# AdamCodd/local-hyperDB

Measured on AMD Instinct MI355X. Metric: queries/sec, N=10M d=384 fp16 top-100 (single-query stream; p50 latency alongside), higher is better.
Workload: dtype f16; 1 GPU; N=10000000 d=384 fp16 Q=1 cosine_similarity top-100, row-sharded x1; rows_per_gpu=10000000, accumulate=f32, exchange=none

## Files before the change

local-hyperdb_amd/csrc/hdb_api.hip:

```cpp
#include "hdb_common.h"
#include "hdb_quant.h"
#include "hdb_ws.h"
#include "hdb_plan.h"
#include "../../include/hyperdb_hip.h"
#include <string>
#include <cmath>
#include <cstring>
#include <cstdio>
#include <algorithm>
#include <vector>
#include <chrono>
#include <atomic>

static thread_local std::string g_err;
static int fail(int code, const std::string& msg) { g_err = msg; return code; }
#define HIP_TRY(expr)                                                                              \
    do {                                                                                           \
        hipError_t e_ = (expr);                                                                    \
        if (e_ != hipSuccess)                                                                      \
            return fail(HDB_ERR_HIP, std::string(#expr) + ": " + hipGetErrorString(e_));           \
    } while (0)
#define LAUNCH_TRY(expr)                                                                           \
    do {                                                                                           \
        int e_ = (expr);                                                                           \
// ... 59 lines not shown
    int64_t profile = 0;
    std::vector<hipEvent_t> ev_pool;
    size_t ev_used = 0;
};

static int ensure_ws(hdb_index* ix, size_t bytes) {
    if (bytes <= ix->ws_bytes) return HDB_OK;
    if (ix->ws) { HIP_TRY(hipDeviceSynchronize()); HIP_TRY(hipFree(ix->ws)); ix->ws = nullptr; ix->ws_bytes = 0; }
    bytes = align_up(bytes + (bytes >> 2), 1 << 20);
    HIP_TRY(hipMalloc((void**)&ix->ws, bytes));
    ix->ws_bytes = bytes;
    return HDB_OK;
}
template <typename WS, typename... Ext>
static int ws_lay(hdb_index* ix, WS& w, Ext... ext) {
    const int rc = ensure_ws(ix, ws_bytes_for<WS>(ext...));
    if (rc) return rc;
    Bump b(ix->ws, ix->ws_bytes);
    w.lay(b, ext...);
    if (b.off > b.cap) return fail(HDB_ERR_NOMEM, "workspace: a layout ran past the size it reported");
    return HDB_OK;
}

extern "C" int hdb_version(void) { return 105; }
extern "C" const char* hdb_last_error(void) { return g_err.c_str(); }

static int build_caches(hdb_index* ix, hipStream_t st) {
    if (ix->n > ix->cache_rows) {
        if (ix->inv_norm) { HIP_TRY(hipDeviceSynchronize()); HIP_TRY(hipFree(ix->inv_norm)); HIP_TRY(hipFree(ix->sqnorm)); }
        const int64_t rows = ix->n + ix->n / 4 + 64;
        HIP_TRY(hipMalloc((void**)&ix->inv_norm, rows * sizeof(float)));
        HIP_TRY(hipMalloc((void**)&ix->sqnorm, rows * sizeof(float)));
        ix->cache_rows = rows;
    }
    HIP_TRY(hipMemsetAsync(ix->nan_flag, 0, sizeof(int), st));
    if (ix->n > 0) LAUNCH_TRY(hdb_launch_rownorm(ix->V, ix->n, ix->d, ix->dtype, ix->inv_norm, ix->sqnorm, ix->nan_flag, st));
    ix->flags_host = -1;
    ix->bits_valid = false; ix->bits_done = 0;
    ix->pscale_valid = false; ix->pscale_done = 0;
    ix->build_stream = st;
    return HDB_OK;
}

static double quant_gamma(int d) {
    const double u = std::ldexp(1.0, -24), m = (double)(d + 8) * u;
    return m / (1.0 - m) * (1.0 + std::ldexp(1.0, -20));
}
// ... 339 lines not shown
    else if (!strcmp(name, "dyn_heavy")) ix->opt.dyn_heavy = value;
    else if (!strcmp(name, "fused_timeout_us")) ix->opt.fused_timeout_us = std::max<int64_t>(1, value);
    else if (!strcmp(name, "bits_fused")) ix->opt.bits_fused = value;
    else if (!strcmp(name, "bits_local")) ix->opt.bits_local = value;
    else if (!strcmp(name, "fused_max_q")) ix->opt.fused_max_q = value;
    else if (!strcmp(name, "f32_min_q")) ix->opt.f32_min_q = value;
    else if (!strcmp(name, "f32_split")) ix->opt.f32_split = value;
    else if (!strcmp(name, "f32_split_min_q")) ix->opt.f32_split_min_q = value;
    else if (!strcmp(name, "bf16_ks_min_q")) ix->opt.bf16_ks_min_q = value;
    else if (!strcmp(name, "f8_ks_min_q")) ix->opt.f8_ks_min_q = value < 0 ? -1 : value;
    else if (!strcmp(name, "f8_lds_min_q")) ix->opt.f8_lds_min_q = value < 0 ? -1 : value;
    else if (!strcmp(name, "bf16_quant")) ix->opt.bf16_quant = value ? 1 : 0;
    else if (!strcmp(name, "f8_lds_waves")) { if (value == 0 || value == 4 || value == 8) ix->opt.f8_lds_waves = value; }
    else if (!strcmp(name, "bits_max_q")) ix->opt.bits_max_q = value;
    else if (!strcmp(name, "use_quant")) ix->opt.use_quant = value;
    else if (!strcmp(name, "quant_min_n")) ix->opt.quant_min_n = value;
    else if (!strcmp(name, "auto_quant")) ix->opt.auto_quant = value;
    else if (!strcmp(name, "quant_batch_min_n")) ix->opt.quant_batch_min_n = value;
    else if (!strcmp(name, "quant_batch_kernel")) ix->opt.quant_batch_kernel = value ? 1 : 0;
    else if (!strcmp(name, "quant_max_k")) ix->opt.quant_max_k = std::max<int64_t>(1, std::min<int64_t>(value, 128));
    else if (!strcmp(name, "use_plane")) ix->opt.use_plane = value;
    else if (!strcmp(name, "plane_min_n")) ix->opt.plane_min_n = value;
    else if (!strcmp(name, "plane_cap_rows")) ix->opt.plane_cap_rows = std::max<int64_t>(0, value);
    else if (!strcmp(name, "use_subset")) ix->opt.use_subset = value;
    else if (!strcmp(name, "subset_min_n")) ix->opt.subset_min_n = value < 0 ? -1 : value;
    else if (!strcmp(name, "subset_ratio")) ix->opt.subset_ratio = value < 0 ? -1 : std::max<int64_t>(1, value);
    else if (!strcmp(name, "profile")) { ix->profile = value; ix->ev_used = 0; }
    else if (!strcmp(name, "host_timing_reset")) { ix->ht_pre_ns = ix->ht_launch_ns = ix->ht_wait_ns = ix->ht_calls = ix->ht_attr_ns = 0; }
    else return fail(HDB_ERR_ARG, std::string("hdb_set_option: unknown option ") + name);
    return HDB_OK;
}

extern "C" int hdb_get_stat(hdb_index* ix, const char* name, int64_t* value) {
    if (!ix || !name || !value) return fail(HDB_ERR_ARG, "hdb_get_stat: null argument");
    if (!strcmp(name, "sample_rows")) *value = ix->st.sample_rows;
    else if (!strcmp(name, "sample_m")) *value = ix->st.sample_m;
    else if (!strcmp(name, "path")) *value = ix->st.path;
    else if (!strcmp(name, "chunks")) *value = ix->st.chunks;
    else if (!strcmp(name, "mfma")) *value = ix->st.mfma;
    else if (!strcmp(name, "f32_split")) *value = ix->st.f32s;
    else if (!strcmp(name, "f8_lds")) *value = ix->st.f8_lds;
    else if (!strcmp(name, "f8_lds_min_q")) *value = f8_lds_first_q(ix->opt, ix->dtype, ix->d);
    else if (!strcmp(name, "host_direct")) *value = ix->st_host_direct;
    else if (!strcmp(name, "fused")) *value = ix->st.fused;
    else if (!strcmp(name, "local")) *value = ix->st.local;
    else if (!strcmp(name, "cand_cap")) *value = HDB_CAND_CAP;
    else if (!strcmp(name, "quant")) *value = ix->st.quant;
    else if (!strcmp(name, "quant_auto")) *value = (ix->qmode == HDB_QUANT_I8 && ix->qauto) ? 1 : 0;
    else if (!strcmp(name, "quant_bytes")) *value = ix->qmode == HDB_QUANT_I8 ? ix->n * (int64_t)(ix->qP + 12) : 0;
    else if (!strcmp(name, "plane")) *value = ix->st.plane;
    else if (!strcmp(name, "subset")) *value = ix->st.subset;
    else if (!strcmp(name, "subset_rows")) *value = ix->subset_m;
    else if (!strcmp(name, "plane_bytes")) *value = (ix->qmode == HDB_QUANT_I8 && ix->pnib) ? ix->n * (int64_t)plane_row_bytes(ix->qP) : 0;
    else if (!strcmp(name, "plane_survivors") || !strcmp(name, "plane_overflows")) {
        int h[HDB_QSTAT_WORDS] = {0, 0, 0, 0};
        if (ix->qstat) {
            HIP_TRY(hipSetDevice(ix->device));
            HIP_TRY(hipDeviceSynchronize());
            HIP_TRY(hipMemcpy(h, ix->qstat, sizeof(h), hipMemcpyDeviceToHost));
        }
        *value = name[6] == 's' ? (ix->st.plane ? (int64_t)(uint32_t)h[1] : 0) : (int64_t)(uint32_t)h[2];
    }
    else if (!strcmp(name, "quant_cands")) {
        int h = 0;
        if (ix->st.quant && ix->qstat) {
            HIP_TRY(hipSetDevice(ix->device));
            HIP_TRY(hipDeviceSynchronize());
            HIP_TRY(hipMemcpy(&h, ix->qstat, sizeof(int), hipMemcpyDeviceToHost));
        }
        *value = h;
    }
    else if (!strcmp(name, "quant_cands_min") || !strcmp(name, "quant_cands_median")) {
        int64_t v = 0;
// ... 211 lines not shown
    const size_t crow = (size_t)nq * HDB_CAND_CAP;
    const int nsub = p.nsub;
    rc = quant_query_prep(ix, (const float*)dev_Q, nq, w, mflavour, ix->qstat, nsub ? w.cnt : nullptr, pl_cnt, st);
    if (rc) return rc;
    QuantArgs a; quant_base_args(ix, a, w.qcodes, w.qaux, w.qinv, metric, nq);
    a.ntiles = sp.s_tiles; a.tile_stride = sp.s_stride; a.scores = w.sbuf; a.ld = sp.ld_s;
    a.wmax = w.wmax; a.nsub = nsub; a.thr_out = w.thr;
    a.pl_hi = use_pl ? reinterpret_cast<float*>(w.pl_list) : nullptr;
    if (use_pl && (!a.pl_hi || sp.s_rows > (int64_t)quant_hi_cap(ix, nq))) return fail(HDB_ERR_ARG, "quant_topk: no list for the sampled rows");
    LAUNCH_TRY(hdb_launch_quant_scan(&a, 0, (int)ix->opt.max_blocks, st));
    if (!nsub) LAUNCH_TRY(hdb_launch_sample_thr(w.sbuf, sp.s_rows, sp.ld_s, nq, m, w.thr, w.cnt, nullptr, st));
    a.ntiles = (n + 15) / 16; a.tile_stride = 1; a.scores = nullptr; a.ld = 0;
    a.thr = w.thr; a.cnt = w.cnt; a.cand = w.cand; a.cap = HDB_CAND_CAP;
    const bool has_bias = ix->bias != nullptr || ix->mask != nullptr;
    if (mflavour) {
        a.V = (const char*)ix->V; a.row_bytes = ix->d * 2; a.G = w.G;
        a.ginv = metric == HDB_COSINE ? w.ginv : nullptr; a.gbias = has_bias ? w.gbias : nullptr;
    }
    prof_begin(ix, st);
    if (use_pl) {
        a.pl_nib = ix->pnib; a.pl_bit = ix->pbit; a.pl_rec = ix->prec; a.pl_units = ix->pU;
        a.pl_cnt = pl_cnt; a.pl_cap = p.pl_cap;
        a.pl_s_tiles = (uint32_t)sp.s_tiles; a.pl_s_stride = (uint32_t)sp.s_stride;
        LAUNCH_TRY(hdb_launch_quant_plane_scan(&a, 0, (int)ix->opt.max_blocks, st));
    } else {
        LAUNCH_TRY(hdb_launch_quant_scan(&a, 1, (int)ix->opt.max_blocks, st));
    }
    prof_end(ix, st);
    if (mflavour) {
        ScanArgs s; memset(&s, 0, sizeof(s));
        s.V = w.G; s.n = (int64_t)crow; s.d = ix->d; s.Q = dev_Q; s.metric = metric; s.inv_norm = w.ginv; s.qinv = w.qinv;
        s.bias = has_bias ? w.gbias : nullptr; s.mask = nullptr; s.nq = nq;
        s.tile_stride = 1; s.ntiles = (int64_t)crow / hdb_mfma_tile_rows(ix->dtype, ix->d); s.cap = HDB_CAND_CAP;
        s.scores = w.gsc; s.ld = (int64_t)crow;
        LAUNCH_TRY(hdb_launch_mfma_scan(&s, ix->dtype, 0, nq, w.q16, w.ginv, w.qsq, w.qscl, (int)ix->opt.max_blocks, (int)ix->opt.mfma_variant, st, nullptr));
    } else {
        LAUNCH_TRY(hdb_launch_quant_rescore(ix->V, ix->d, ix->dtype, (const float*)dev_Q, nq, metric, ix->inv_norm, w.qinv, ix->bias, ix->mask,
                                            w.cand, w.cnt, HDB_CAND_CAP, st));
    }
    LAUNCH_TRY(hdb_launch_quant_finalize(w.cand, w.cnt, HDB_CAND_CAP, nq, (uint32_t)k, kk, ix->row_base, dev_idx, dev_score, dev_status, w.qnan,
                                         w.qaux, w.thr, ix->qstat, mflavour ? w.cand : nullptr, w.gsc, (int64_t)crow, st));
    return HDB_OK;
}

extern "C" int hdb_debug_quant_bounds(hdb_index* ix, const float* dev_q, int metric, float* dev_hi, float* dev_hi5, void* stream) {
    if (!ix || !dev_q || !dev_hi || !dev_hi5) return fail(HDB_ERR_ARG, "hdb_debug_quant_bounds: null argument");
    if (metric != HDB_DOT && metric != HDB_COSINE) return fail(HDB_ERR_ARG, "hdb_debug_quant_bounds: dot or cosine");
    if (ix->qmode != HDB_QUANT_I8 || !ix->pnib || ix->n < 1) return fail(HDB_ERR_UNSUPPORTED, "hdb_debug_quant_bounds: the index has no 5-bit plane");
    HIP_TRY(hipSetDevice(ix->device));
    hipStream_t st = (hipStream_t)stream;
    QuantWs w;
    int rc = quant_ws_lay(ix, w, 1, quant_hi_cap(ix, 1), true);
    if (rc) return rc;
    rc = quant_query_prep(ix, dev_q, 1, w, ix->qauto, nullptr, nullptr, nullptr, st);
    if (rc) return rc;
    QuantArgs a; quant_base_args(ix, a, w.qcodes, w.qaux, w.qinv, metric, 1);
    a.ntiles = (ix->n + 15) / 16; a.tile_stride = 1;
    a.pl_nib = ix->pnib; a.pl_bit = ix->pbit; a.pl_rec = ix->prec; a.pl_units = ix->pU;
    a.dbg = dev_hi;
    LAUNCH_TRY(hdb_launch_quant_scan_one(&a, 2, (int)ix->opt.max_blocks, st));
    a.dbg = dev_hi5;
    LAUNCH_TRY(hdb_launch_quant_plane_scan(&a, 1, (int)ix->opt.max_blocks, st));
    return HDB_OK;
}

static int quant_batch_topk(hdb_index* ix, const TopkArgs& c, const TopkPlan& p) {
    const void* dev_Q = c.Q; const int32_t nq = c.nq, k = c.k; const int metric = c.metric; hipStream_t st = c.st;
    int64_t* dev_idx = c.idx; float* dev_score = c.score; int32_t* dev_status = c.status;
    const uint32_t kk = p.kk;
    const int64_t n = ix->n;
    const int P = ix->qP;
    const uint32_t m = HDB_QB_SAMPLE_M;
    const QuantSample sp = p.qs;
    const int64_t s_tiles = sp.s_tiles, s_stride = sp.s_stride, s_rows = sp.s_rows, ld_s = sp.ld_s;
    const int cq_max = p.cq_max;
    QuantBatchWs w;
    const int rc = quant_batch_ws_lay(ix, w, cq_max);
    if (rc) return rc;
    const int64_t wld = quant_batch_wld();
    float* const qinv = w.qinv; float* const qsq = w.qsq; int* const qnan = w.qnan; float* const qscl = w.qscl;
    int8_t* const qcodes = w.qcodes; float* const qaux = w.qaux; float* const thr = w.thr; uint32_t* const cnt = w.cnt;
    unsigned long long* const cand = w.cand; void* const q16 = w.q16; float* const wbuf = w.wbuf;
    for (int q0 = 0; q0 < nq; q0 += cq_max) {
        const int cq = std::min(cq_max, nq - q0);
        const float* Qc = (const float*)dev_Q + (size_t)q0 * ix->d;
// ... 673 lines not shown
```

local-hyperdb_amd/csrc/hdb_caps.h:

```cpp
#pragma once
#include "../../include/hyperdb_hip.h"

static inline int hdb_scan_auto_blocks(int dtype, int row_bytes, bool vec, bool wide_rows) {
    if (dtype == HDB_F8E4M3 && vec && (row_bytes == 256 || row_bytes == 384 || row_bytes == 512)) {
        const int b = 512 * 768 / row_bytes;
        return b < 1024 ? b : 1024;
    }
    return wide_rows ? 256 : 512;
}

#define HDB_KS_MAX_SLICES 8
struct KsGeom {
    int slices;
    int width[HDB_KS_MAX_SLICES];
    int off[HDB_KS_MAX_SLICES];
};
static inline KsGeom ks_list(int elem_bytes, int n0, int w0, int n1 = 0, int w1 = 0) {
    KsGeom g = {};
    int at = 0;
    for (int s = 0; s < n0 + n1 && s < HDB_KS_MAX_SLICES; ++s) {
        g.width[s] = s < n0 ? w0 : w1; g.off[s] = at * elem_bytes;
        at += g.width[s];
    }
    g.slices = n0 + n1;
// ... 137 lines not shown
#endif
#define HDB_BITS_MAXW 512
static inline int hdb_bits_fused_supported(int metric, int nq, int W, uint32_t kk) {
    return (metric == HDB_HAMMING || metric == HDB_JACCARD) && nq >= 1 && nq <= 4 && W <= HDB_BITS_MAXW && kk <= 128;
}
static inline int hdb_bits_fused_blocks(int64_t ntiles, int cus, int max_blocks) {
    int blocks = cus;
    const int64_t items = ntiles * 4;
    if ((int64_t)blocks * HDB_BITS_THREADS > items) blocks = (int)((items + HDB_BITS_THREADS - 1) / HDB_BITS_THREADS);
    if (max_blocks > 0 && max_blocks < blocks) blocks = max_blocks;
    if (blocks < 1) blocks = 1;
    return blocks;
}
static inline bool hdb_bits_fused_local(int blocks, uint32_t kk) { return (int64_t)blocks >= 2 * (int64_t)kk; }

static inline int hdb_l1_tile_supported(int dtype, int d) {
    if (dtype == HDB_F16) return d == 128 || d == 256 || d == 384 || d == 512 || d == 640 || d == 768;
    if (dtype == HDB_F32) return d == 128 || d == 256 || d == 384 || d == 512 || d == 768;
    return 0;
}

static inline int hdb_quant_scan_blocks(int64_t ntiles, int max_blocks) { return hdb_grid_for(ntiles, 4, max_blocks > 0 ? max_blocks : 1024); }
static inline int hdb_quant_plane_units(int P) { return (P + 31) / 32; }
struct HdbSkipPos { uint32_t w, o; };
struct HdbSkipStep { uint32_t dw, dn, step; };
__host__ __device__ __forceinline__ uint32_t hdb_plane_skip_count(uint32_t ntiles, uint32_t s_tiles) { return ntiles - s_tiles; }
__host__ __device__ __forceinline__ HdbSkipStep hdb_plane_skip_step(uint32_t step, uint32_t stride) {
    const uint32_t m = stride - 1u;
    HdbSkipStep s;
    s.dw = m ? step / m : 0u; s.dn = m ? step % m : 0u; s.step = step;
    return s;
}
__host__ __device__ __forceinline__ HdbSkipPos hdb_plane_skip_start(uint32_t tp, uint32_t s_tiles, uint32_t stride) {
    const uint32_t m = stride - 1u;
    HdbSkipPos p;
    const uint32_t w = m ? tp / m : s_tiles;
    if (w < s_tiles) { p.w = w; p.o = tp - w * m; }
    else { p.w = s_tiles; p.o = tp - s_tiles * m; }
    return p;
}
__host__ __device__ __forceinline__ void hdb_plane_skip_advance(HdbSkipPos& p, const HdbSkipStep& s, uint32_t s_tiles, uint32_t stride) {
    if (p.w >= s_tiles) { p.o += s.step; return; }
    const uint32_t m = stride - 1u;
    p.w += s.dw; p.o += s.dn;
    if (p.o >= m) { p.o -= m; ++p.w; }
    if (p.w >= s_tiles) { p.o += (p.w - s_tiles) * m; p.w = s_tiles; }
// ... 20 lines not shown
```

local-hyperdb_amd/csrc/hdb_launch.h:

```cpp
#pragma once
#include <stddef.h>
#include <stdint.h>

struct ScanArgs;
struct FusedArgs;
struct BatchArgs;
struct BitsArgs;
struct QuantArgs;

#define HDB_ANYD_DECL(name) int name(const ScanArgs* args, int dpad, int mode, int nq_launch, const void* q, const float* sqnorm, \
                                     const float* qsq, const float* qscl, int blocks, void* stream)
#define HDB_GEOM_DECL(name) int name(const ScanArgs* args, int mode, int nq_launch, const void* q16, const float* sqnorm, \
                                     const float* qsq, const float* qscl, int blocks, int variant, void* stream, const BatchArgs* f)

extern "C" {
int hdb_launch_scan(const ScanArgs* args, int dtype, int mode, int nq_launch, int max_blocks, void* stream);
int hdb_launch_list_rows(unsigned long long* cand, const uint32_t* cnt, uint32_t cap, int nq, const int64_t* rows, int64_t m, void* stream);
int hdb_launch_rownorm(const void* V, int64_t n, int d, int dtype, float* inv_norm, float* sqnorm, int* nan_flag, void* stream);
int hdb_launch_qprep(const void* Q, int nq, int d, bool f64, float* qinv, float* qsq, int* qnan, void* q16, float* qscl, void* stream);
int hdb_launch_qprep2(const void* Q, int nq, int d, bool f64, float* qinv, float* qsq, int* qnan, void* q16, float* qscl,
                      float* thr_init, uint32_t* cnt_init, uint32_t* qbits, int W, void* stream);
int hdb_launch_signpack(const void* V, int64_t n, int d, int dtype, int64_t row0, uint32_t* bits, void* stream);
int hdb_launch_qsign(const void* Q, int nq, int d, bool f64, int W, uint32_t* qbits, void* stream);
int hdb_launch_hamming(const ScanArgs* args, int mode, int nq_launch, const uint32_t* bits, int64_t npad, int W,
// ... 72 lines not shown
int hdb_launch_mfma_kslice_f8_lds(const ScanArgs* a, int dslice, int mode, int nq_launch, const void* q, const float* sqnorm,
                                  const float* qsq, int blocks, void* stream);
int hdb_launch_mfma_kslice_f8_lds_wide(const ScanArgs* a, int dslice, int mode, int nq_launch, const void* q, const float* sqnorm,
                                       const float* qsq, int blocks, void* stream);
HDB_ANYD_DECL(hdb_launch_mfma_anyd_a); HDB_ANYD_DECL(hdb_launch_mfma_anyd_b);
HDB_ANYD_DECL(hdb_launch_mfma_anyd_c); HDB_ANYD_DECL(hdb_launch_mfma_anyd_d);
HDB_ANYD_DECL(hdb_launch_mfma_anyd_e); HDB_ANYD_DECL(hdb_launch_mfma_anyd_f);

size_t hdb_mfma_fused_ctl_bytes(void);
int hdb_launch_mfma_fused(const ScanArgs* args, int dtype, const FusedArgs* fa, int max_blocks, void* stream);
int hdb_launch_mfma_fused_wide(const ScanArgs* args, const FusedArgs* fa, int blocks, void* stream);
int hdb_launch_bits_fused(const BitsArgs* args, int jaccard, int max_blocks, void* stream);
int hdb_launch_l1_tile(const ScanArgs* args, int dtype, int mode, int nq_launch, int max_blocks, void* stream);

int hdb_launch_quant_rows(const void* V, int64_t n, int d, int dtype, int P, int8_t* codes, float* aux, int* nan_flag, double gamma,
                          void* stream);
int hdb_launch_quant_gather(const int8_t* codes, const float* aux, const int64_t* rows, int64_t m, int P, int8_t* codes_out,
                            float* aux_out, void* stream);
int hdb_launch_quant_qprep(const float* Q, int nq, int d, int P, int8_t* qcodes, float* qaux, int* stat, uint32_t* pl_cnt, void* stream);
int hdb_launch_quant_qprep_m(const float* Q, int nq, int d, int P, float* qinv, float* qsq, int* qnan, void* q16, float* qscl,
                             int8_t* qcodes, float* qaux, int* stat, uint32_t* cnt_init, uint32_t* pl_cnt, void* stream);
int hdb_launch_quant_plane_rows(const int8_t* codes, const float* aux, int64_t row0, int64_t m, int d, int P, uint8_t* nib, uint32_t* bitw,
                                float* rec, void* stream);
int hdb_launch_quant_plane_scan(const QuantArgs* args, int dbg, int max_blocks, void* stream);
int hdb_launch_quant_scan(const QuantArgs* args, int mode, int max_blocks, void* stream);
int hdb_launch_quant_scan_one(const QuantArgs* args, int mode, int max_blocks, void* stream);
int hdb_launch_quant_rescore(const void* V, int d, int dtype, const float* Q, int nq, int metric, const float* inv_norm,
                             const float* qinv, const float* bias, const uint8_t* mask, unsigned long long* cand,
                             const uint32_t* cnt, uint32_t cap, void* stream);
int hdb_launch_quant_finalize(const unsigned long long* cand, const uint32_t* cnt, uint32_t cap, int nq, uint32_t k, uint32_t kk,
                              int64_t row_base, int64_t* idx_out, float* score_out, int32_t* status, const int* qnan,
                              const float* qaux, const float* thr, int* stat, unsigned long long* cand_rw, const float* sc, int64_t ld,
                              void* stream);

int hdb_launch_qb_scan(const QuantArgs* args, int mode, float* wstat, int64_t wld, int max_blocks, void* stream);
int hdb_launch_qb_thr(const float* vals, int64_t n, int64_t ld, int nq, uint32_t m, float* thr, void* stream);
int hdb_launch_qb_rescore(const void* V, int d, const void* q16, const float* qscl, const float* qinv, const float* inv_norm,
                          const float* bias, const uint8_t* mask, int metric, unsigned long long* cand, const uint32_t* cnt,
                          uint32_t cap, int nq, void* stream);
}
```

local-hyperdb_amd/csrc/hdb_plan.h:

```cpp
#pragma once
#include "hdb_ws.h"
#include <algorithm>

struct hdb_options {
    int64_t max_blocks = 0;
    int64_t force_exact = 0;
    int64_t sample_target = 0;
    int64_t mfma_min_q = 1;
    int64_t use_mfma = 1;
    int64_t exact_bytes = (int64_t)1 << 30;
    int64_t bits_fused = 1;
    int64_t bits_local = 1;
    int64_t fused_max_q = -1;
    int64_t f32_min_q = -1;
    int64_t f32_split = 1;
    int64_t f32_split_min_q = -1;
    int64_t bf16_ks_min_q = -1;
    int64_t f8_ks_min_q = 0;
    int64_t f8_lds_min_q = 0;
    int64_t bf16_quant = 0;
    int64_t f8_lds_waves = 0;
    int64_t bits_max_q = -1;
    int64_t host_direct = 1;
    int64_t dyn_tiles = 1;
// ... 1 lines not shown
    int64_t dyn_heavy = 0;
    int64_t host_poll = 1;
    int64_t use_fused = 1;
    int64_t use_local = 1;
    int64_t local_m = 0;
    int64_t local_max_tiles = 4;
    int64_t local_small = 0;
    int64_t local_max_q = 1;
    int64_t use_l1_tile = 1;
    int64_t l1_packed = 1;
    int64_t use_batch1 = 1;
    int64_t fused_timeout_us = 2000;
    int64_t finalize_threads = 1024;
    int64_t mfma_variant = 16;
    int64_t use_quant = 1;
    int64_t quant_min_n = -1;
    int64_t quant_max_k = 128;
    int64_t auto_quant = 1;
    int64_t quant_batch_min_n = -1;
    int64_t quant_batch_kernel = 1;
    int64_t use_plane = 1;
    int64_t plane_min_n = -1;
    int64_t plane_cap_rows = 0;
    int64_t use_subset = 1;
    int64_t subset_min_n = -1;
    int64_t subset_ratio = -1;
};

struct TopkFacts {
    int64_t n; int32_t d; int dtype;
    int qmode;
    bool qauto;
    bool qauto_declined;
    bool plane_present, plane_declined;
    bool has_mask, has_bias;
    int cus;
    int64_t subset_m;
};
struct TopkCall { int32_t nq, k; int metric; bool has_status, exact; };

enum TopkPath {
    HDB_PATH_EMPTY,
    HDB_PATH_QUANT,
    HDB_PATH_QUANT_BATCH,
    HDB_PATH_FUSED,
    HDB_PATH_BITS1,
    HDB_PATH_BATCH1,
    HDB_PATH_FULL_SORT,
    HDB_PATH_PIPELINE
};
struct TopkStats { int64_t sample_rows = 0, sample_m = 0, path = 0, chunks = 0, mfma = 0, fused = 0, local = 0, f32s = 0, quant = 0, plane = 0, subset = 0, f8_lds = 0; };
struct TopkPlan {
    TopkPath path = HDB_PATH_EMPTY;
    uint32_t kk = 0; int W = 0;
    bool bits = false, pearson = false;
    bool exact = false, small = false, mfma = false, f32s = false, ksplit = false, l1tile = false, local = false;
    bool f8_lds = false;
    bool subset = false;
    bool prep = false, fold_small = false, q16_in_prep = false, f16_queries = false, mask_fold = false;
    int tile_rows = 16;
    int64_t s_tiles = 0, s_stride = 1, s_rows = 0, ld_s = 0, ld_n = 0; uint32_t m = 0;
    int cq_max = 1;
    int64_t ld_scores = 0, ld_ks = 0, sort_n = 0;
    uint32_t local_slot = 0, local_m = 0;
    int bits_local = 0;
    int npass = 4;
    bool mflavour = false, build_needed = false, plane_wanted = false;
    bool qb_int8 = false;
    int P = 0, nsub = 0; uint32_t pl_cap = 0;
    QuantSample qs = {0, 1, 0, 0};
    TopkStats stats;
    bool shadow() const { return path == HDB_PATH_QUANT || path == HDB_PATH_QUANT_BATCH; }
    bool single_launch() const { return path == HDB_PATH_FUSED || path == HDB_PATH_BITS1 || path == HDB_PATH_BATCH1; }
};

#define HDB_FUSED_MAXQ_RULE 4
static inline bool is_bits_metric(int metric) { return metric == HDB_HAMMING || metric == HDB_JACCARD; }

static inline void sample_plan(int64_t n, int64_t sample_target, uint32_t kk, int nq, int tile_rows, bool coarse, int64_t& tiles, int64_t& stride, uint32_t& m) {
    int64_t T = sample_target > 0 ? sample_target : (kk <= 128 ? (nq >= 32 ? 1024 : 2048) : 4096);
    if (coarse && sample_target <= 0) T /= 2;
    m = kk <= 128 ? 8u : (kk <= 512 ? 64u : 256u);
    int64_t rows = (int64_t)((double)m * (double)n / (double)T);
    rows = std::max<int64_t>(rows, 16 * (int64_t)m);
    tiles = (rows + tile_rows - 1) / tile_rows;
    const int64_t all_tiles = n / tile_rows;
    tiles = std::min(tiles, all_tiles);
    stride = std::max<int64_t>(1, all_tiles / std::max<int64_t>(tiles, 1));
}

static inline int64_t quant_min_rows(int dtype) {
    return dtype == HDB_F16 ? 1250000 : dtype == HDB_BF16 ? 1000000 : 500000;
// ... 8 lines not shown
static inline bool plane_wanted(int d, const hdb_options& o) { return plane_possible(d) && o.use_plane; }

static inline int64_t quant_batch_rule(int d, int nq) {
    int64_t rows = 0;
    if (d == 384) rows = nq <= 16 ? 3000000 : nq <= 24 ? 5000000 : 0;
    else if (d == 512) rows = nq <= 16 ? 10000000 : 0;
    return rows > 0 ? std::max<int64_t>(rows, HDB_QUANT_AUTO_MIN_ROWS) : 0;
}
static inline int64_t quant_batch_wld() { return (int64_t)align_up((size_t)hdb_qb_slots(512, 1), 4); }

static inline bool auto_quant_call(const TopkFacts& ix, const hdb_options& o, const TopkCall& c, bool mfma, bool exact, bool small) {
    return o.auto_quant && o.use_quant && mfma && ix.dtype == HDB_F16 && (ix.qmode == HDB_QUANT_NONE || ix.qauto) && !exact && !small &&
           c.has_status && c.k <= o.quant_max_k && c.k <= 128 && (c.metric == HDB_DOT || c.metric == HDB_COSINE) &&
           !(ix.qmode == HDB_QUANT_NONE && ix.qauto_declined);
}

static inline void plan_quant(TopkPlan& p, const TopkFacts& ix, const hdb_options& o, const TopkCall& c, bool mflavour) {
    p.path = HDB_PATH_QUANT; p.mflavour = mflavour; p.build_needed = ix.qmode != HDB_QUANT_I8;
    p.P = (int)align_up((size_t)ix.d, 16);
    p.qs = quant_call_sample(ix.n, ix.d, p.kk);
    p.plane_wanted = c.nq == 1 && (c.metric == HDB_DOT || c.metric == HDB_COSINE) && plane_wanted(ix.d, o) && !ix.plane_declined &&
                     ix.n >= (o.plane_min_n >= 0 ? o.plane_min_n : (int64_t)HDB_PLANE_MIN_ROWS);
    p.pl_cap = plane_list_cap(o, ix.n);
    if (mflavour) {
        p.nsub = 4 * hdb_quant_scan_blocks(p.qs.s_tiles, (int)o.max_blocks);
        if (p.nsub < 1024 || p.nsub > HDB_QUANT_NSUB_MAX) p.nsub = 0;
    }
    p.stats.quant = 1; p.stats.path = 1; p.stats.mfma = mflavour ? 1 : 0; p.stats.plane = p.plane_wanted ? 1 : 0;
    p.stats.sample_rows = p.qs.s_rows; p.stats.sample_m = 16; p.stats.chunks = 1;
}
static inline void plan_quant_batch(TopkPlan& p, const TopkFacts& ix, const hdb_options& o, const TopkCall& c) {
    p.path = HDB_PATH_QUANT_BATCH; p.mflavour = true; p.build_needed = ix.qmode != HDB_QUANT_I8;
    p.P = (int)align_up((size_t)ix.d, 16);
    p.qs = quant_batch_sample(ix.n);
    p.cq_max = std::min<int>(c.nq, 256);
    p.qb_int8 = o.quant_batch_kernel != 0;
    p.stats.quant = 1; p.stats.path = 1; p.stats.mfma = 1;
    p.stats.sample_rows = p.qs.s_rows; p.stats.sample_m = HDB_QB_SAMPLE_M; p.stats.chunks = (c.nq + p.cq_max - 1) / p.cq_max;
}

#define HDB_SUBSET_RATIO 4
#define HDB_SUBSET_MIN_ROWS 50000
static inline bool subset_metric(int metric) {
    return metric == HDB_DOT || metric == HDB_COSINE || metric == HDB_EUCLIDEAN || metric == HDB_MANHATTAN || metric == HDB_PEARSON;
}
static inline bool subset_rule(const TopkFacts& ix, const hdb_options& o, const TopkCall& c) {
    if (ix.subset_m <= 0 || !o.use_subset || !subset_metric(c.metric) || c.nq < 1) return false;
    if (ix.n < (o.subset_min_n >= 0 ? o.subset_min_n : (int64_t)HDB_SUBSET_MIN_ROWS)) return false;
    const int64_t ratio = o.subset_ratio >= 1 ? std::min<int64_t>(o.subset_ratio, (int64_t)1 << 30) : (int64_t)HDB_SUBSET_RATIO;
    return ix.subset_m <= ix.n / (((int64_t)c.nq + 3) / 4 * ratio);
}
// ... 143 lines not shown
```

local-hyperdb_amd/csrc/hdb_quant.hip:

```cpp
#include "hdb_common.h"
#include "hdb_quant.h"
#include "hdb_finalize.h"
#include "../../include/hyperdb_hip.h"

__device__ __forceinline__ float hq_up(double x) {
    x = x * (1.0 + 0x1p-40);
    float f = (float)x;
    if ((double)f < x) f = nextafterf(f, INFINITY);
    return f;
}

__device__ __forceinline__ float hq_f(__half v) { return __half2float(v); }
__device__ __forceinline__ float hq_f(hdb_bf16 v) { return hdb_bf16_to_f(v); }
__device__ __forceinline__ float hq_f(float v) { return v; }

template <typename T> struct HqElem;
template <> struct HqElem<__half> { static constexpr int EPC = 8; };
template <> struct HqElem<hdb_bf16> { static constexpr int EPC = 8; };
template <> struct HqElem<float> { static constexpr int EPC = 4; };

__device__ __forceinline__ void hq_unpack(const uint4& raw, float (&x)[8], __half*) {
    const __half2* h = reinterpret_cast<const __half2*>(&raw);
#pragma unroll
    for (int i = 0; i < 4; ++i) { float2 f = __half22float2(h[i]); x[2 * i] = f.x; x[2 * i + 1] = f.y; }
// ... 538 lines not shown
    extern __shared__ __attribute__((aligned(16))) char smem[];
    int4* qs = reinterpret_cast<int4*>(smem);
    __shared__ int part[4][2][64 * J];
    __shared__ HqStage stage;
    __shared__ uint32_t queue[4][HQ_PL_QUEUE];
    __shared__ uint32_t surv_cnt;
    const int U = a.pl_units, nch = a.P >> 4;
    if (threadIdx.x < 4) stage.cnt[threadIdx.x] = 0u;
    if (threadIdx.x == 0) surv_cnt = 0u;
    for (int i = threadIdx.x; i < 2 * U; i += 256) qs[i] = i < nch ? reinterpret_cast<const int4*>(a.qcodes)[i] : make_int4(0, 0, 0, 0);
    const float* qo = a.qaux;
    const float q_s = qo[HDB_QQ_S], q_n = qo[HDB_QQ_N], q_d = qo[HDB_QQ_D], q_cn = qo[HDB_QQ_CN];
    const int q_cs = (int)qo[HDB_QQ_CS];
    const bool q_bad = qo[HDB_QQ_BAD] != 0.f;
    const bool cosine = a.metric == HDB_COSINE;
    const float q_inv = cosine ? a.qinv[0] : 1.f;
    float thr1[1] = {(!DBG && a.nsub == 0) ? a.thr[0] : 0.f};
    __syncthreads();
    if (!DBG && a.nsub > 0) hq_fold_thr<1>(a, thr1);
    const float q_thr = thr1[0];

    const int lane = threadIdx.x & 63, wave = __builtin_amdgcn_readfirstlane(threadIdx.x >> 6);
    const int npieces = 16 * U;
    int qw[J][8];
    auto load_qw = [&]() {
#pragma unroll
        for (int j = 0; j < J; ++j) {
            const int f = lane + 64 * j;
            const int unit = f < npieces ? f % U : 0;
            const int4 x = qs[2 * unit], y = qs[2 * unit + 1];
            qw[j][0] = x.x; qw[j][1] = x.y; qw[j][2] = x.z; qw[j][3] = x.w;
            qw[j][4] = y.x; qw[j][5] = y.y; qw[j][6] = y.z; qw[j][7] = y.w;
        }
    };
    load_qw();
    const float absmin = 0x1p-100f * (float)(a.d + 8);
    typedef unsigned int u32x4 __attribute__((ext_vector_type(4)));
    typedef float f32x4 __attribute__((ext_vector_type(4)));
    const int64_t ntiles = a.ntiles;
    const int et = lane >> 4, er = lane & 15;
    int qn = 0;
    uint32_t nsurv = 0u;
    auto drain = [&](int base, int m) {
        const QuantArgs& a = hq_args_in_memory();
        HqQuery<1> qc;
        qc.s[0] = q_s; qc.n[0] = q_n; qc.d[0] = q_d; qc.sq[0] = 0.f; qc.inv[0] = q_inv; qc.bad[0] = q_bad;
        int ln = lane;
        asm volatile("" : "+v"(ln));
        const int g = ln >> 4, l16 = ln & 15;
        int64_t rr[4];
#pragma unroll
        for (int u = 0; u < 4; ++u) rr[u] = 4 * g + u < m ? (int64_t)queue[wave][base + 4 * g + u] : a.n;
        const int own = 4 * g + hdb_owned_row(l16);
        const int64_t row = own < m ? (int64_t)queue[wave][base + own] : a.n;
        hq_rows4_bounds<1, 0, 1>(a, qs, qc, rr, l16, row, [&](int, float, float hi, bool masked) {
            if (!masked && !q_bad && hi >= q_thr) hq_emit(stage, 0, hi, row);
        });
    };
// ... 24 lines not shown
            for (int j = 0; j < J; ++j) {
                if (ln < pieces_left - 64 * j) {
                    nv[tt][j] = __builtin_nontemporal_load(reinterpret_cast<const u32x4*>(nb + (uint32_t)ln * 16u) + 64 * j);
                    bv[tt][j] = __builtin_nontemporal_load(bb + (uint32_t)ln + 64 * j);
                } else {
                    nv[tt][j] = u32x4{0u, 0u, 0u, 0u};
                    bv[tt][j] = 0u;
                }
            }
        }
        const int64_t row = (et ? tl[1] : tl[0]) * 16 + er;
        const bool rvalid = lane < 32 && row < a.n;
        f32x4 rc = f32x4{0.f, 0.f, 0.f, 0.f};
        float invn = 1.f, bias = 0.f;
        bool masked = false;
        if (rvalid) {
            rc = __builtin_nontemporal_load(reinterpret_cast<const f32x4*>(a.pl_rec) + row);
            if (cosine) invn = a.inv_norm[row];
            if (a.bias) bias = a.bias[row];
            if (a.mask) masked = !a.mask[row];
        }
        __builtin_amdgcn_sched_barrier(0);
#pragma unroll
        for (int tt = 0; tt < 2; ++tt) {
#pragma unroll
            for (int j = 0; j < J; ++j) {
                const uint32_t bw = bv[tt][j];
                const uint32_t w4[4] = {nv[tt][j].x, nv[tt][j].y, nv[tt][j].z, nv[tt][j].w};
                int s = 0;
#pragma unroll
                for (int i = 0; i < 4; ++i) {
                    const uint32_t lo = ((w4[i] << 1) & 0x1E1E1E1Eu) | ((bw >> (2 * i)) & 0x01010101u);
                    const uint32_t hi = ((w4[i] >> 3) & 0x1E1E1E1Eu) | ((bw >> (2 * i + 1)) & 0x01010101u);
                    s = __builtin_amdgcn_sdot4((int)lo, qw[j][2 * i], s, false);
                    s = __builtin_amdgcn_sdot4((int)hi, qw[j][2 * i + 1], s, false);
                }
                part[wave][tt][lane + 64 * j] = s;
            }
        }
        __builtin_amdgcn_fence(__ATOMIC_RELEASE, "wavefront");
        __builtin_amdgcn_wave_barrier();
        __builtin_amdgcn_fence(__ATOMIC_ACQUIRE, "wavefront");
        int S = 0;
        if (lane < 32)
            for (int i = 0; i < U; ++i) S += part[wave][et][er * U + i];
        __builtin_amdgcn_fence(__ATOMIC_RELEASE, "wavefront");
        __builtin_amdgcn_wave_barrier();
        float hi5 = -INFINITY;
        const bool dead = !rvalid || masked || q_bad;
        if (!dead) {
            const float fc = (float)(8 * S - 124 * q_cs);
            const float Uf = q_cn * rc.w;
            float ch = fc + Uf, cl = fc - Uf;
            ch = ch + (fabsf(ch) * 0x1p-20f + 1.f);
            cl = cl - (fabsf(cl) * 0x1p-20f + 1.f);
            const float k = q_s * rc.x;
            const float A5 = k * ch, Al = k * cl;
            const float Amax = fmaxf(fabsf(A5), fabsf(Al));
            const float c0 = (q_n * rc.y + q_d * rc.z) * (1.f + 0x1p-10f);
            const float B5 = c0 + fabsf(A5) * 0x1p-10f + absmin;
            const float Bmax = c0 + Amax * 0x1p-10f + absmin;
// ... 4 lines not shown
            const float Z = mM + fabsf(bias);
            float h = X;
            if (a.bias) h += bias;
            hi5 = h + (Z * 0x1p-18f + 4e-30f);
            if (hi5 != hi5) hi5 = INFINITY;
        }
        if (DBG) {
            if (rvalid) a.dbg[row] = hi5;
            continue;
        }
        const bool keep = !dead && !(hi5 < q_thr);
        const unsigned long long km = __ballot(keep);
        if (km == 0ull) continue;
        if (keep) queue[wave][qn + __popcll(km & ((1ull << lane) - 1ull))] = (uint32_t)row;
        const int nk = __popcll(km);
        qn += nk; nsurv += (uint32_t)nk;
        __builtin_amdgcn_fence(__ATOMIC_RELEASE, "wavefront");
        __builtin_amdgcn_wave_barrier();
        __builtin_amdgcn_fence(__ATOMIC_ACQUIRE, "wavefront");
        if (qn >= 16) {
            do { qn -= 16; drain(qn, 16); } while (qn >= 16);
            __builtin_amdgcn_fence(__ATOMIC_RELEASE, "wavefront");
            __builtin_amdgcn_wave_barrier();
            asm volatile("" ::: "memory");
            load_qw();
        }
    }
    if (!DBG) {
        if (s_tiles != 0u) {
            const QuantArgs& am = hq_args_in_memory();
            const uint32_t nslots = s_tiles * 16u, dslot = (uint32_t)gridDim.x * 256u;
            uint32_t cbase = ((uint32_t)blockIdx.x * 4u + (uint32_t)wave) * 64u;
            float hnext = cbase + lane < nslots ? am.pl_hi[cbase + lane] : 0.f;
#pragma unroll 1
            for (; cbase < nslots; cbase += dslot) {
                const uint32_t slot = cbase + lane;
                const float hi = hnext;
                hnext = slot + dslot < nslots ? am.pl_hi[slot + dslot] : 0.f;
                const int64_t row = hdb_tile_index((int64_t)(slot >> 4), (int64_t)s_stride) * 16 + (slot & 15u);
                bool keep = slot < nslots && !q_bad && !(hi < q_thr);
                if (keep && am.mask) keep = am.mask[row] != 0;
                const unsigned long long km = __ballot(keep);
#pragma unroll 1
                for (int h = 0; h < 2; ++h) {
                    const uint32_t kh = (uint32_t)(km >> (32 * h));
                    if (kh == 0u) continue;
                    if (keep && (lane >> 5) == h) queue[wave][qn + __popc(kh & ((1u << (lane & 31)) - 1u))] = (uint32_t)row;
                    const int nk = __popc(kh);
// ... 172 lines not shown
extern "C" int hdb_launch_quant_scan(const QuantArgs* args, int mode, int max_blocks, void* stream) {
    const QuantArgs& a = *args;
    if (a.nq < 1 || a.nq > 4 || (a.P & 15) != 0) return (int)hipErrorInvalidValue;
    const size_t lds = (size_t)a.nq * a.P;
    const int blocks = hdb_quant_scan_blocks(a.ntiles, max_blocks);
    if (a.nsub != 0 && (a.nsub > HDB_QUANT_NSUB_MAX || !a.wmax || (mode == 0 ? a.nsub != 4 * blocks : !a.thr_out))) return (int)hipErrorInvalidValue;
    if (mode == 0) hq_launch_scan_mode<0>(a, blocks, lds, (hipStream_t)stream);
    else {
        if (!hq_copy_args_ok(a)) return (int)hipErrorInvalidValue;
        hq_launch_scan_mode<1>(a, blocks, lds, (hipStream_t)stream);
    }
    return (int)hipGetLastError();
}

extern "C" int hdb_launch_quant_plane_rows(const int8_t* codes, const float* aux, int64_t row0, int64_t m, int d, int P, uint8_t* nib,
                                           uint32_t* bitw, float* rec, void* stream) {
    if (m <= 0) return 0;
    const int U = hdb_quant_plane_units(P);
    if (U > 16 || (P & 15) != 0) return (int)hipErrorInvalidValue;
    hipLaunchKernelGGL(hdb_quant_plane_rows_kernel, dim3(hdb_grid_for(m, 16, 8192)), dim3(256), 0, (hipStream_t)stream, codes, aux, row0, m, d,
                       P, U, nib, bitw, rec);
    return (int)hipGetLastError();
}
extern "C" int hdb_launch_quant_plane_scan(const QuantArgs* args, int dbg, int max_blocks, void* stream) {
    const QuantArgs& a = *args;
    const int U = a.pl_units;
    if (a.nq != 1 || U < 1 || U > 16 || U != hdb_quant_plane_units(a.P) || (a.metric != HDB_DOT && a.metric != HDB_COSINE)) return (int)hipErrorInvalidValue;
    if (!dbg && a.nsub != 0 && (a.nsub > HDB_QUANT_NSUB_MAX || !a.wmax || !a.thr_out)) return (int)hipErrorInvalidValue;
    if (!dbg && (!a.cnt || !a.cand || !a.pl_cnt || !hq_copy_args_ok(a))) return (int)hipErrorInvalidValue;
    if (a.ntiles < 0 || a.ntiles > 0x10000000) return (int)hipErrorInvalidValue;
    if (!dbg && a.pl_s_tiles != 0u && (!a.pl_hi || a.pl_s_stride < 1u || (uint64_t)a.pl_s_tiles * a.pl_s_stride > (uint64_t)a.ntiles)) return (int)hipErrorInvalidValue;
    const size_t lds = (size_t)U * 32;
    const int64_t nwalk = a.ntiles - (dbg ? 0 : (int64_t)a.pl_s_tiles);
    const int blocks = hdb_grid_for((nwalk + 1) / 2, 4, max_blocks > 0 ? max_blocks : 1024);
    hipStream_t st = (hipStream_t)stream;
    const int J = (U + 3) / 4;
#define HQ_PLANE(J_) do { if (dbg) hipLaunchKernelGGL((hdb_quant_plane_scan_kernel<J_, true>), dim3(blocks), dim3(256), lds, st, a); \
                          else hipLaunchKernelGGL((hdb_quant_plane_scan_kernel<J_, false>), dim3(blocks), dim3(256), lds, st, a); } while (0)
    if (J == 1) HQ_PLANE(1); else if (J == 2) HQ_PLANE(2); else if (J == 3) HQ_PLANE(3); else HQ_PLANE(4);
#undef HQ_PLANE
    return (int)hipGetLastError();
}
extern "C" int hdb_launch_quant_scan_one(const QuantArgs* args, int mode, int max_blocks, void* stream) {
    const QuantArgs& a = *args;
    if (a.nq != 1 || (a.P & 15) != 0 || a.nsub != 0 || mode != 2 || !a.dbg) return (int)hipErrorInvalidValue;
    const size_t lds = (size_t)a.P;
    const int blocks = hdb_quant_scan_blocks(a.ntiles, max_blocks);
    const int nj = ((a.P >> 4) + 15) >> 4;
    hipStream_t st = (hipStream_t)stream;
#define HQ_ONE(NJ_) hipLaunchKernelGGL((hdb_quant_scan_kernel<2, 1, NJ_>), dim3(blocks), dim3(256), lds, st, a)
    if (nj == 1) HQ_ONE(1); else if (nj == 2) HQ_ONE(2); else if (nj == 3) HQ_ONE(3); else HQ_ONE(0);
#undef HQ_ONE
    return (int)hipGetLastError();
}

extern "C" int hdb_launch_quant_rescore(const void* V, int d, int dtype, const float* Q, int nq, int metric, const float* inv_norm,
                                        const float* qinv, const float* bias, const uint8_t* mask, unsigned long long* cand,
                                        const uint32_t* cnt, uint32_t cap, void* stream) {
    hipStream_t st = (hipStream_t)stream;
// ... 39 lines not shown
```

Measured before the change: 1997 queries/s.

## Size plane-scan grid per CU and load query words from LDS per use

```diff
diff --git a/local-hyperdb_amd/csrc/hdb_api.hip b/local-hyperdb_amd/csrc/hdb_api.hip
--- a/local-hyperdb_amd/csrc/hdb_api.hip
+++ b/local-hyperdb_amd/csrc/hdb_api.hip
@@ -105,7 +105,7 @@
     return HDB_OK;
 }
 
-extern "C" int hdb_version(void) { return 105; }
+extern "C" int hdb_version(void) { return 106; }
 extern "C" const char* hdb_last_error(void) { return g_err.c_str(); }
 
 static int build_caches(hdb_index* ix, hipStream_t st) {
@@ -491,6 +491,7 @@
     else if (!strcmp(name, "use_plane")) ix->opt.use_plane = value;
     else if (!strcmp(name, "plane_min_n")) ix->opt.plane_min_n = value;
     else if (!strcmp(name, "plane_cap_rows")) ix->opt.plane_cap_rows = std::max<int64_t>(0, value);
+    else if (!strcmp(name, "plane_wg_per_cu")) ix->opt.plane_wg_per_cu = std::max<int64_t>(0, std::min<int64_t>(value, 8));
     else if (!strcmp(name, "use_subset")) ix->opt.use_subset = value;
     else if (!strcmp(name, "subset_min_n")) ix->opt.subset_min_n = value < 0 ? -1 : value;
     else if (!strcmp(name, "subset_ratio")) ix->opt.subset_ratio = value < 0 ? -1 : std::max<int64_t>(1, value);
@@ -518,6 +519,7 @@
     else if (!strcmp(name, "quant_auto")) *value = (ix->qmode == HDB_QUANT_I8 && ix->qauto) ? 1 : 0;
     else if (!strcmp(name, "quant_bytes")) *value = ix->qmode == HDB_QUANT_I8 ? ix->n * (int64_t)(ix->qP + 12) : 0;
     else if (!strcmp(name, "plane")) *value = ix->st.plane;
+    else if (!strcmp(name, "plane_blocks")) *value = ix->st.plane_blocks;
     else if (!strcmp(name, "subset")) *value = ix->st.subset;
     else if (!strcmp(name, "subset_rows")) *value = ix->subset_m;
     else if (!strcmp(name, "plane_bytes")) *value = (ix->qmode == HDB_QUANT_I8 && ix->pnib) ? ix->n * (int64_t)plane_row_bytes(ix->qP) : 0;
@@ -775,7 +777,7 @@
         a.pl_nib = ix->pnib; a.pl_bit = ix->pbit; a.pl_rec = ix->prec; a.pl_units = ix->pU;
         a.pl_cnt = pl_cnt; a.pl_cap = p.pl_cap;
         a.pl_s_tiles = (uint32_t)sp.s_tiles; a.pl_s_stride = (uint32_t)sp.s_stride;
-        LAUNCH_TRY(hdb_launch_quant_plane_scan(&a, 0, (int)ix->opt.max_blocks, st));
+        LAUNCH_TRY(hdb_launch_quant_plane_scan(&a, 0, p.pl_blocks, st));
     } else {
         LAUNCH_TRY(hdb_launch_quant_scan(&a, 1, (int)ix->opt.max_blocks, st));
     }
@@ -813,7 +815,7 @@
     a.dbg = dev_hi;
     LAUNCH_TRY(hdb_launch_quant_scan_one(&a, 2, (int)ix->opt.max_blocks, st));
     a.dbg = dev_hi5;
-    LAUNCH_TRY(hdb_launch_quant_plane_scan(&a, 1, (int)ix->opt.max_blocks, st));
+    LAUNCH_TRY(hdb_launch_quant_plane_scan(&a, 1, hdb_quant_plane_dbg_blocks(a.ntiles, (int)ix->opt.max_blocks), st));
     return HDB_OK;
 }
 
diff --git a/local-hyperdb_amd/csrc/hdb_caps.h b/local-hyperdb_amd/csrc/hdb_caps.h
--- a/local-hyperdb_amd/csrc/hdb_caps.h
+++ b/local-hyperdb_amd/csrc/hdb_caps.h
@@ -183,6 +183,23 @@
 
 static inline int hdb_quant_scan_blocks(int64_t ntiles, int max_blocks) { return hdb_grid_for(ntiles, 4, max_blocks > 0 ? max_blocks : 1024); }
 static inline int hdb_quant_plane_units(int P) { return (P + 31) / 32; }
+static constexpr int hdb_quant_plane_j(int U) { return (U + 3) / 4; }
+#define HDB_PLANE_WAVES {8, 8, 7, 5}
+#define HDB_PLANE_WG_PER_CU {4, 4, 3, 2}
+static constexpr int hdb_quant_plane_waves(int J) { constexpr int t[4] = HDB_PLANE_WAVES; return t[J < 1 ? 0 : J > 4 ? 3 : J - 1]; }
+static constexpr int hdb_quant_plane_wg_per_cu(int J) { constexpr int t[4] = HDB_PLANE_WG_PER_CU; return t[J < 1 ? 0 : J > 4 ? 3 : J - 1]; }
+static_assert(hdb_quant_plane_wg_per_cu(1) >= 1 && hdb_quant_plane_wg_per_cu(1) <= hdb_quant_plane_waves(1) &&
+              hdb_quant_plane_wg_per_cu(2) >= 1 && hdb_quant_plane_wg_per_cu(2) <= hdb_quant_plane_waves(2) &&
+              hdb_quant_plane_wg_per_cu(3) >= 1 && hdb_quant_plane_wg_per_cu(3) <= hdb_quant_plane_waves(3) &&
+              hdb_quant_plane_wg_per_cu(4) >= 1 && hdb_quant_plane_wg_per_cu(4) <= hdb_quant_plane_waves(4),
+              "a default grid of the plane pass asks for more waves per SIMD than its kernel is compiled for");
+static inline int hdb_quant_plane_blocks(int64_t nwalk, int J, int cus, int wg_per_cu, int max_blocks) {
+    const int per_cu = wg_per_cu >= 1 ? (wg_per_cu < 8 ? wg_per_cu : 8) : hdb_quant_plane_wg_per_cu(J);
+    int64_t limit = (int64_t)per_cu * (cus > 0 ? cus : 1);
+    if (max_blocks > 0 && max_blocks < limit) limit = max_blocks;
+    return hdb_grid_for((nwalk + 1) / 2, 4, (int)limit);
+}
+static inline int hdb_quant_plane_dbg_blocks(int64_t ntiles, int max_blocks) { return hdb_grid_for((ntiles + 1) / 2, 4, max_blocks > 0 ? max_blocks : 1024); }
 struct HdbSkipPos { uint32_t w, o; };
 struct HdbSkipStep { uint32_t dw, dn, step; };
 __host__ __device__ __forceinline__ uint32_t hdb_plane_skip_count(uint32_t ntiles, uint32_t s_tiles) { return ntiles - s_tiles; }
diff --git a/local-hyperdb_amd/csrc/hdb_launch.h b/local-hyperdb_amd/csrc/hdb_launch.h
--- a/local-hyperdb_amd/csrc/hdb_launch.h
+++ b/local-hyperdb_amd/csrc/hdb_launch.h
@@ -118,7 +118,7 @@
                              int8_t* qcodes, float* qaux, int* stat, uint32_t* cnt_init, uint32_t* pl_cnt, void* stream);
 int hdb_launch_quant_plane_rows(const int8_t* codes, const float* aux, int64_t row0, int64_t m, int d, int P, uint8_t* nib, uint32_t* bitw,
                                 float* rec, void* stream);
-int hdb_launch_quant_plane_scan(const QuantArgs* args, int dbg, int max_blocks, void* stream);
+int hdb_launch_quant_plane_scan(const QuantArgs* args, int dbg, int blocks, void* stream);
 int hdb_launch_quant_scan(const QuantArgs* args, int mode, int max_blocks, void* stream);
 int hdb_launch_quant_scan_one(const QuantArgs* args, int mode, int max_blocks, void* stream);
 int hdb_launch_quant_rescore(const void* V, int d, int dtype, const float* Q, int nq, int metric, const float* inv_norm,
diff --git a/local-hyperdb_amd/csrc/hdb_plan.h b/local-hyperdb_amd/csrc/hdb_plan.h
--- a/local-hyperdb_amd/csrc/hdb_plan.h
+++ b/local-hyperdb_amd/csrc/hdb_plan.h
@@ -47,6 +47,7 @@
     int64_t use_plane = 1;
     int64_t plane_min_n = -1;
     int64_t plane_cap_rows = 0;
+    int64_t plane_wg_per_cu = 0;
     int64_t use_subset = 1;
     int64_t subset_min_n = -1;
     int64_t subset_ratio = -1;
@@ -74,7 +75,7 @@
     HDB_PATH_FULL_SORT,
     HDB_PATH_PIPELINE
 };
-struct TopkStats { int64_t sample_rows = 0, sample_m = 0, path = 0, chunks = 0, mfma = 0, fused = 0, local = 0, f32s = 0, quant = 0, plane = 0, subset = 0, f8_lds = 0; };
+struct TopkStats { int64_t sample_rows = 0, sample_m = 0, path = 0, chunks = 0, mfma = 0, fused = 0, local = 0, f32s = 0, quant = 0, plane = 0, subset = 0, f8_lds = 0, plane_blocks = 0; };
 struct TopkPlan {
     TopkPath path = HDB_PATH_EMPTY;
     uint32_t kk = 0; int W = 0;
@@ -93,6 +94,7 @@
     bool mflavour = false, build_needed = false, plane_wanted = false;
     bool qb_int8 = false;
     int P = 0, nsub = 0; uint32_t pl_cap = 0;
+    int pl_blocks = 0;
     QuantSample qs = {0, 1, 0, 0};
     TopkStats stats;
     bool shadow() const { return path == HDB_PATH_QUANT || path == HDB_PATH_QUANT_BATCH; }
@@ -147,11 +149,15 @@
     p.plane_wanted = c.nq == 1 && (c.metric == HDB_DOT || c.metric == HDB_COSINE) && plane_wanted(ix.d, o) && !ix.plane_declined &&
                      ix.n >= (o.plane_min_n >= 0 ? o.plane_min_n : (int64_t)HDB_PLANE_MIN_ROWS);
     p.pl_cap = plane_list_cap(o, ix.n);
+    if (p.plane_wanted)
+        p.pl_blocks = hdb_quant_plane_blocks((ix.n + 15) / 16 - p.qs.s_tiles, hdb_quant_plane_j(hdb_quant_plane_units(p.P)), ix.cus,
+                                             (int)o.plane_wg_per_cu, (int)o.max_blocks);
     if (mflavour) {
         p.nsub = 4 * hdb_quant_scan_blocks(p.qs.s_tiles, (int)o.max_blocks);
         if (p.nsub < 1024 || p.nsub > HDB_QUANT_NSUB_MAX) p.nsub = 0;
     }
     p.stats.quant = 1; p.stats.path = 1; p.stats.mfma = mflavour ? 1 : 0; p.stats.plane = p.plane_wanted ? 1 : 0;
+    p.stats.plane_blocks = p.pl_blocks;
     p.stats.sample_rows = p.qs.s_rows; p.stats.sample_m = 16; p.stats.chunks = 1;
 }
 static inline void plan_quant_batch(TopkPlan& p, const TopkFacts& ix, const hdb_options& o, const TopkCall& c) {
diff --git a/local-hyperdb_amd/csrc/hdb_quant.hip b/local-hyperdb_amd/csrc/hdb_quant.hip
--- a/local-hyperdb_amd/csrc/hdb_quant.hip
+++ b/local-hyperdb_amd/csrc/hdb_quant.hip
@@ -584,18 +584,12 @@
 
     const int lane = threadIdx.x & 63, wave = __builtin_amdgcn_readfirstlane(threadIdx.x >> 6);
     const int npieces = 16 * U;
-    int qw[J][8];
-    auto load_qw = [&]() {
-#pragma unroll
-        for (int j = 0; j < J; ++j) {
-            const int f = lane + 64 * j;
-            const int unit = f < npieces ? f % U : 0;
-            const int4 x = qs[2 * unit], y = qs[2 * unit + 1];
-            qw[j][0] = x.x; qw[j][1] = x.y; qw[j][2] = x.z; qw[j][3] = x.w;
-            qw[j][4] = y.x; qw[j][5] = y.y; qw[j][6] = y.z; qw[j][7] = y.w;
-        }
-    };
-    load_qw();
+    int qoff[J];
+#pragma unroll
+    for (int j = 0; j < J; ++j) {
+        const int f = lane + 64 * j;
+        qoff[j] = f < npieces ? 2 * (f % U) : 0;
+    }
     const float absmin = 0x1p-100f * (float)(a.d + 8);
     typedef unsigned int u32x4 __attribute__((ext_vector_type(4)));
     typedef float f32x4 __attribute__((ext_vector_type(4)));
@@ -666,9 +660,11 @@
         }
         __builtin_amdgcn_sched_barrier(0);
 #pragma unroll
-        for (int tt = 0; tt < 2; ++tt) {
-#pragma unroll
-            for (int j = 0; j < J; ++j) {
+        for (int j = 0; j < J; ++j) {
+            const int4 x = qs[qoff[j]], y = qs[qoff[j] + 1];
+            const int qw[8] = {x.x, x.y, x.z, x.w, y.x, y.y, y.z, y.w};
+#pragma unroll
+            for (int tt = 0; tt < 2; ++tt) {
                 const uint32_t bw = bv[tt][j];
                 const uint32_t w4[4] = {nv[tt][j].x, nv[tt][j].y, nv[tt][j].z, nv[tt][j].w};
                 int s = 0;
@@ -676,11 +672,12 @@
                 for (int i = 0; i < 4; ++i) {
                     const uint32_t lo = ((w4[i] << 1) & 0x1E1E1E1Eu) | ((bw >> (2 * i)) & 0x01010101u);
                     const uint32_t hi = ((w4[i] >> 3) & 0x1E1E1E1Eu) | ((bw >> (2 * i + 1)) & 0x01010101u);
-                    s = __builtin_amdgcn_sdot4((int)lo, qw[j][2 * i], s, false);
-                    s = __builtin_amdgcn_sdot4((int)hi, qw[j][2 * i + 1], s, false);
+                    s = __builtin_amdgcn_sdot4((int)lo, qw[2 * i], s, false);
+                    s = __builtin_amdgcn_sdot4((int)hi, qw[2 * i + 1], s, false);
                 }
                 part[wave][tt][lane + 64 * j] = s;
             }
+            __builtin_amdgcn_sched_barrier(0);
         }
         __builtin_amdgcn_fence(__ATOMIC_RELEASE, "wavefront");
         __builtin_amdgcn_wave_barrier();
@@ -731,8 +728,6 @@
             do { qn -= 16; drain(qn, 16); } while (qn >= 16);
             __builtin_amdgcn_fence(__ATOMIC_RELEASE, "wavefront");
             __builtin_amdgcn_wave_barrier();
-            asm volatile("" ::: "memory");
-            load_qw();
         }
     }
     if (!DBG) {
@@ -951,19 +946,18 @@
                        P, U, nib, bitw, rec);
     return (int)hipGetLastError();
 }
-extern "C" int hdb_launch_quant_plane_scan(const QuantArgs* args, int dbg, int max_blocks, void* stream) {
+extern "C" int hdb_launch_quant_plane_scan(const QuantArgs* args, int dbg, int blocks, void* stream) {
     const QuantArgs& a = *args;
     const int U = a.pl_units;
+    if (blocks < 1 || blocks > (1 << 22)) return (int)hipErrorInvalidValue;
     if (a.nq != 1 || U < 1 || U > 16 || U != hdb_quant_plane_units(a.P) || (a.metric != HDB_DOT && a.metric != HDB_COSINE)) return (int)hipErrorInvalidValue;
     if (!dbg && a.nsub != 0 && (a.nsub > HDB_QUANT_NSUB_MAX || !a.wmax || !a.thr_out)) return (int)hipErrorInvalidValue;
     if (!dbg && (!a.cnt || !a.cand || !a.pl_cnt || !hq_copy_args_ok(a))) return (int)hipErrorInvalidValue;
     if (a.ntiles < 0 || a.ntiles > 0x10000000) return (int)hipErrorInvalidValue;
     if (!dbg && a.pl_s_tiles != 0u && (!a.pl_hi || a.pl_s_stride < 1u || (uint64_t)a.pl_s_tiles * a.pl_s_stride > (uint64_t)a.ntiles)) return (int)hipErrorInvalidValue;
     const size_t lds = (size_t)U * 32;
-    const int64_t nwalk = a.ntiles - (dbg ? 0 : (int64_t)a.pl_s_tiles);
-    const int blocks = hdb_grid_for((nwalk + 1) / 2, 4, max_blocks > 0 ? max_blocks : 1024);
     hipStream_t st = (hipStream_t)stream;
-    const int J = (U + 3) / 4;
+    const int J = hdb_quant_plane_j(U);
 #define HQ_PLANE(J_) do { if (dbg) hipLaunchKernelGGL((hdb_quant_plane_scan_kernel<J_, true>), dim3(blocks), dim3(256), lds, st, a); \
                           else hipLaunchKernelGGL((hdb_quant_plane_scan_kernel<J_, false>), dim3(blocks), dim3(256), lds, st, a); } while (0)
     if (J == 1) HQ_PLANE(1); else if (J == 2) HQ_PLANE(2); else if (J == 3) HQ_PLANE(3); else HQ_PLANE(4);
```

After: 2054 queries/s (median of 6 runs). 1.03x the previous value.
